# endernewton/tf-faster-rcnn

Hardware: AMD Instinct MI355X
Metric: images/sec (600×1000) ResNet-101 Faster R-CNN at 1/2/4/8 MI355X (higher is better)
Workload: dtype f32 (operands, accumulators, results; GEMMs with Cin, Cout % 128 == 0 form each f32 product from two-piece fp16 operands with an exact power-of-two scale per 128-k block on the fp16 matrix pipe -- 3 MFMAs / product, dropped terms <= 3 * 2^-22, measured error vs float64 below the f32-MFMA kernel's; o

## Files before the change

tf-faster-rcnn_amd/csrc/conv_igemm.hip:

```cpp
#include "common.h"
#include "mfma_f32.h"
#include <mutex>
#include <type_traits>

__device__ float4 g_zero_page[4];

struct ConvParams {
  const float* x; const float* w; const float* bias; const float* res; float* y;
  const float* mask;
  int N, H, W, Cin, OH, OW, Cout, KH, KW, stride, pad_top, pad_left, act;
  int RH, RW, res_stride;
  int M, Ktot, nsteps;
  int mtiles, ntiles;
  int batch;
  long long gx, gw, gy;
  int reserved;
  int splits, kchunk;
  long long gz;
  int stagger, stagger_slots;
};

__device__ __forceinline__ size_t res_offset_strided(int m, int n, int Cout, int res_stride, int ohow, int OW, int RH, int RW) {
  const int img = m / ohow, rem = m % ohow, oh = rem / OW, ow = rem % OW;
  return ((size_t)(img * RH + oh * res_stride) * RW + ow * res_stride) * Cout + n;
}

template <int TM, int TN>
__device__ __forceinline__ void frag_read(float4 (&a)[TM], const float* sb, const int& a_row0, const int& koff, float4 (&b)[TN], const int& b_row0) {
#pragma unroll
  for (int i = 0; i < TM; ++i) a[i] = *(const float4*)(sb + a_row0 + i * 1024 + koff);
#pragma unroll
  for (int j = 0; j < TN; ++j) b[j] = *(const float4*)(sb + b_row0 + j * 1024 + koff);
}
template <int TM, int TN>
__device__ __forceinline__ void frag_mfma(const float4 (&a)[TM], const float4 (&b)[TN], f32x16 (&acc2)[TM][TN], f32x16 (&acc)[TM][TN]) {
  constexpr bool KSPLIT = (TM * TN == 1);
#pragma unroll
  for (int e = 0; e < 4; ++e)
#pragma unroll
    for (int i = 0; i < TM; ++i)
#pragma unroll
      for (int j = 0; j < TN; ++j) {
        const float av = e == 0 ? a[i].x : e == 1 ? a[i].y : e == 2 ? a[i].z : a[i].w;
        const float bv = e == 0 ? b[j].x : e == 1 ? b[j].y : e == 2 ? b[j].z : b[j].w;
        if (KSPLIT && (e & 1)) acc2[i][j] = __builtin_amdgcn_mfma_f32_32x32x2f32(av, bv, acc2[i][j], 0, 0, 0);
        else acc[i][j] = __builtin_amdgcn_mfma_f32_32x32x2f32(av, bv, acc[i][j], 0, 0, 0);
      }
}

template <int BM, int BN, int WM, int WN, int NS, bool FOLDW, bool ILV = false, bool RF = false>
__global__ __launch_bounds__((BM / WM) * (BN / WN) * 64) void k_conv_igemm(const ConvParams p) {
  constexpr int NW = (BM / WM) * (BN / WN);
  constexpr int NT = NW * 64;
  constexpr int TM = WM / 32, TN = WN / 32;
  constexpr int LA = BM / 8 / NW, LB = BN / 8 / NW;
  constexpr int G = LA + LB;
  constexpr int P = NS - 1;
  constexpr int SLAB = (BM + BN) * 32;
  constexpr int EPI_LD = BN;
  static_assert((BM / 8) % NW == 0 && (BN / 8) % NW == 0, "tile/wave mismatch");
  static_assert((P - 1) * G <= 63, "vmcnt range");
  extern __shared__ __attribute__((aligned(16))) float smem[];

  const int tid = threadIdx.x, lane = tid & 63;
  const int wave = __builtin_amdgcn_readfirstlane(tid >> 6);
  if (p.stagger > 0) {
    const unsigned slot = blockIdx.x >> 8;
    if (blockIdx.y == 0 && blockIdx.z == 0 && slot > 0 && slot < (unsigned)p.stagger_slots) {
      const long long t0 = clock64(), wait = (long long)p.stagger * slot;
      while (clock64() - t0 < wait) __builtin_amdgcn_s_sleep(16);
    }
  }
  const int nwg = p.mtiles * p.ntiles;
  int bid = blockIdx.x;
  {
    const int q = nwg / 8, r = nwg % 8, xcd = bid % 8, idx = bid / 8;
    bid = (xcd < r ? xcd * (q + 1) : r * (q + 1) + (xcd - r) * q) + idx;
  }
  const int mt = bid / p.ntiles, nt = bid % p.ntiles;
  const int bm0 = mt * BM, bn0 = nt * BN;
  const int wm0 = (wave / (BN / WN)) * WM, wn0 = (wave % (BN / WN)) * WN;
  const float* const px = p.x + (size_t)blockIdx.y * p.gx;
  const float* const pw = p.w + (size_t)blockIdx.y * p.gw;
  float* const py = p.y + (size_t)blockIdx.y * p.gy + (size_t)blockIdx.z * p.gz;
  const int s_begin = (int)blockIdx.z * p.kchunk;
  const int nloc = p.splits > 1 ? min(p.nsteps - s_begin, p.kchunk) : p.nsteps;

  const int lrow = lane >> 3, lpos = lane & 7;
  int a_base[LA], a_ih0[LA], a_iw0[LA], a_q4[LA];
#pragma unroll
  for (int t = 0; t < LA; ++t) {
    const int row = (wave * LA + t) * 8 + lrow;
    a_q4[t] = (lpos ^ ((row >> 1) & 7)) * 4;
    const int m = bm0 + row;
    if (m < p.M) {
      const int img = m / (p.OH * p.OW), rem = m % (p.OH * p.OW);
      const int oh = rem / p.OW, ow = rem % p.OW;
      a_base[t] = img * p.H * p.W * p.Cin;
      a_ih0[t] = oh * p.stride - p.pad_top;
      a_iw0[t] = ow * p.stride - p.pad_left;
    } else {
      a_base[t] = 0; a_ih0[t] = -(1 << 28); a_iw0[t] = -(1 << 28);
    }
  }
  const float* zero = (const float*)g_zero_page;
  const float* a_ptr[LA]; int a_inc[LA];
  const float* b_ptr[LB]; int b_inc[LB];
#pragma unroll
  for (int t = 0; t < LB; ++t) {
    const int row = BM + (wave * LB + t) * 8 + lrow;
    const int n = bn0 + row - BM;
    const int q4 = (lpos ^ ((row >> 1) & 7)) * 4;
    const bool ok = n < p.Cout;
    b_ptr[t] = ok ? pw + (size_t)n * p.Ktot + q4 + (size_t)s_begin * 32 : zero;
    b_inc[t] = ok ? 32 : 0;
  }
  int kh = 0, kw = 0, c0 = 0;
  if (!FOLDW && s_begin) {
    const int k0 = s_begin * 32, tap = k0 / p.Cin;
    c0 = k0 - tap * p.Cin;
    kh = tap / p.KW;
    kw = tap - kh * p.KW;
  }

  auto set_tap = [&]() {
#pragma unroll
    for (int t = 0; t < LA; ++t) {
      const int ih = a_ih0[t] + kh, iw = a_iw0[t] + kw;
      bool ok = (unsigned)ih < (unsigned)p.H;
      if (FOLDW) ok = ok && ((unsigned)(iw + (a_q4[t] >> 2)) < (unsigned)p.W);
      else ok = ok && ((unsigned)iw < (unsigned)p.W);
      a_ptr[t] = ok ? px + (size_t)(a_base[t] + (ih * p.W + iw) * p.Cin + c0 + a_q4[t]) : zero;
      a_inc[t] = ok ? 32 : 0;
    }
  };
  const unsigned lds0 = (unsigned)(size_t)(LDS_AS float*)smem;
  auto issue_one = [&](int buf, int t) {
    const unsigned sb = lds0 + (unsigned)(buf * SLAB * 4);
    if (t < LA) {
      glds16(a_ptr[t], __builtin_amdgcn_readfirstlane(sb + (wave * LA + t) * 1024));
      a_ptr[t] += a_inc[t];
    } else {
      const int u = t - LA;
      glds16(b_ptr[u], __builtin_amdgcn_readfirstlane(sb + BM * 128 + (wave * LB + u) * 1024));
      b_ptr[u] += b_inc[u];
    }
  };
  auto advance_k = [&]() {
    if (FOLDW) { ++kh; }
    else {
      c0 += 32;
      if (c0 == p.Cin) { c0 = 0; if (++kw == p.KW) { kw = 0; ++kh; } }
    }
  };
  auto issue_slab = [&](int buf) {
    if (c0 == 0) set_tap();
#pragma unroll
    for (int t = 0; t < G; ++t) issue_one(buf, t);
    advance_k();
  };

  constexpr bool KSPLIT = (TM * TN == 1);
  f32x16 acc[TM][TN], acc2[TM][TN];
#pragma unroll
  for (int i = 0; i < TM; ++i)
#pragma unroll
    for (int j = 0; j < TN; ++j)
#pragma unroll
      for (int r = 0; r < 16; ++r) { acc[i][j][r] = 0.f; acc2[i][j][r] = 0.f; }

  const int frow = lane & 31, khalf = lane >> 5;
  int koff[4];
#pragma unroll
  for (int s = 0; s < 4; ++s) koff[s] = ((2 * s + khalf) ^ ((frow >> 1) & 7)) * 4;
  const int a_row0 = (wm0 + frow) * 32, b_row0 = (BM + wn0 + frow) * 32;

  if (c0 != 0) set_tap();
#pragma unroll
  for (int s = 0; s < P; ++s)
    if (s < nloc) issue_slab(s);

  auto slab = [&](auto more_c, int step) {
    constexpr bool MORE = decltype(more_c)::value;
    if (MORE || step + P <= nloc) wait_vmcnt<(P - 1) * G>();
    else wait_vmcnt<0>();
    __builtin_amdgcn_s_barrier();
    const int nbuf = (step + P) % NS;
    const float* sb = smem + (step % NS) * SLAB;
    float4 a[4][TM], b[4][TN];
    auto read_frag = [&](int q) { frag_read(a[q], sb, a_row0, koff[q], b[q], b_row0); };
    auto mfma_group = [&](int q) { frag_mfma(a[q], b[q], acc2, acc); };
    if (ILV) {
      if (MORE && c0 == 0) set_tap();
      read_frag(0);
#pragma unroll
      for (int q = 0; q < 4; ++q) {
        if (q < 3) read_frag(q + 1);
        if (MORE) {
#pragma unroll
          for (int t = (q * G) / 4; t < ((q + 1) * G) / 4; ++t) issue_one(nbuf, t);
        }
        mfma_group(q);
      }
      if (MORE) advance_k();
    } else {
      constexpr int RF_FIRST = !RF ? 0 : (TM * TN == 1 ? 4 : 1);
#pragma unroll
      for (int q = 0; q < RF_FIRST; ++q) read_frag(q);
      if (MORE) issue_slab(nbuf);
#pragma unroll
      for (int q = RF_FIRST; q < 4; ++q) read_frag(q);
      if (TM * TN == 1) __builtin_amdgcn_sched_barrier(0);
#pragma unroll
      for (int q = 0; q < 4; ++q) mfma_group(q);
    }
  };
  {
    int step = 0;
    for (; step + P < nloc; ++step) slab(std::true_type{}, step);
    for (; step < nloc; ++step) slab(std::false_type{}, step);
  }
  if (KSPLIT) {
#pragma unroll
    for (int i = 0; i < TM; ++i)
#pragma unroll
      for (int j = 0; j < TN; ++j)
#pragma unroll
        for (int r = 0; r < 16; ++r) acc[i][j][r] += acc2[i][j][r];
  }

  __syncthreads();
#pragma unroll
  for (int i = 0; i < TM; ++i)
#pragma unroll
    for (int j = 0; j < TN; ++j)
#pragma unroll
      for (int r = 0; r < 16; ++r) {
        const int ml = wm0 + i * 32 + (r & 3) + 8 * (r >> 2) + 4 * khalf;
        smem[ml * EPI_LD + wn0 + j * 32 + frow] = acc[i][j][r];
      }
  __syncthreads();
  const int ohow = p.OH * p.OW;
  if ((p.Cout & 3) == 0) {
    constexpr int C4 = BN / 4;
    for (int t = tid; t < BM * C4; t += NT) {
      const int ml = t / C4, nl = (t % C4) * 4;
      const int m = bm0 + ml, n = bn0 + nl;
      if (m >= p.M || n >= p.Cout) continue;
      float4 v = *(const float4*)(smem + ml * EPI_LD + nl);
      if (p.bias) {
        const float4 bv = *(const float4*)(p.bias + n);
        v.x += bv.x; v.y += bv.y; v.z += bv.z; v.w += bv.w;
      }
      if (p.res) {
        size_t ro;
        if (p.res_stride == 1) ro = (size_t)m * p.Cout + n;
        else ro = res_offset_strided(m, n, p.Cout, p.res_stride, ohow, p.OW, p.RH, p.RW);
        const float4 rv = *(const float4*)(p.res + ro);
        v.x += rv.x; v.y += rv.y; v.z += rv.z; v.w += rv.w;
      }
      if (p.act == FRCNN_ACT_RELU) v = act_relu(v);
      else if (p.act == FRCNN_ACT_RELU6)
        v = act_relu6(v);
      if (p.mask) {
        const float4 k = *(const float4*)(p.mask + (size_t)m * p.Cout + n);
        v.x = k.x > 0.f ? v.x : 0.f; v.y = k.y > 0.f ? v.y : 0.f; v.z = k.z > 0.f ? v.z : 0.f; v.w = k.w > 0.f ? v.w : 0.f;
      }
      *(float4*)(py + (size_t)m * p.Cout + n) = v;
    }
  } else {
    for (int t = tid; t < BM * BN; t += NT) {
      const int ml = t / BN, nl = t % BN;
      const int m = bm0 + ml, n = bn0 + nl;
      if (m >= p.M || n >= p.Cout) continue;
      float v = smem[ml * EPI_LD + nl] + (p.bias ? p.bias[n] : 0.f);
      if (p.res) {
        size_t ro;
        if (p.res_stride == 1) ro = (size_t)m * p.Cout + n;
        else ro = res_offset_strided(m, n, p.Cout, p.res_stride, ohow, p.OW, p.RH, p.RW);
        v += p.res[ro];
      }
      if (p.act == FRCNN_ACT_RELU) v = act_relu(v);
      else if (p.act == FRCNN_ACT_RELU6) v = act_relu6(v);
      if (p.mask) v = p.mask[(size_t)m * p.Cout + n] > 0.f ? v : 0.f;
      py[(size_t)m * p.Cout + n] = v;
    }
  }
}

template <int BM, int BN, int WM, int WN, int NS, bool FOLDW, bool ILV = false, bool RF = false>
static int launch_conv(ConvParams p, hipStream_t st) {
  constexpr int NT = (BM / WM) * (BN / WN) * 64;
  constexpr size_t ring = sizeof(float) * NS * (BM + BN) * 32, epi = sizeof(float) * BM * BN;
  constexpr size_t lds = ring > epi ? ring : epi;
  auto kern = k_conv_igemm<BM, BN, WM, WN, NS, FOLDW, ILV, RF>;
  static KernelOnce once;
  HIP_TRY(kernel_once(once, (const void*)kern, NT, lds));
  p.mtiles = cdiv(p.M, BM);
  p.ntiles = cdiv(p.Cout, BN);
  hipLaunchKernelGGL(kern, dim3(p.mtiles * p.ntiles, p.batch, p.splits), dim3(NT), lds, st, p);
  LAUNCH_CHECK();
  return FRCNN_OK;
}

struct GemmParams {
  const float* x; const float* w; const float* bias; const float* res; float* y;
  int M, N, K, nsteps, mtiles, ntiles, batch, act;
  long long gx, gw, gy;
};

template <int BM, int BN, int WM, int WN, bool ILV, bool RF, bool RESPF>
__global__ __launch_bounds__((BM / WM) * (BN / WN) * 64) void k_gemm_stream(const GemmParams p) {
  constexpr int NW = (BM / WM) * (BN / WN);
  constexpr int TM = WM / 32, TN = WN / 32;
  constexpr int LA = BM / 8 / NW, LB = BN / 8 / NW;
  constexpr int G = LA + LB;
  constexpr int SLAB = (BM + BN) * 32;
  static_assert((BM / 8) % NW == 0 && (BN / 8) % NW == 0, "tile/wave mismatch");
  extern __shared__ __attribute__((aligned(16))) float smem[];

  const int tid = threadIdx.x, lane = tid & 63;
  const int wave = __builtin_amdgcn_readfirstlane(tid >> 6);
  const int per = p.mtiles * p.ntiles, T = per * p.batch;
  const int xcd = blockIdx.x & 7, wx = blockIdx.x >> 3, W8 = gridDim.x >> 3;
  const int tq = T / 8, tr = T % 8, tn = tq + (xcd < tr ? 1 : 0);
  const int t_end = (xcd < tr ? xcd * (tq + 1) : tr * (tq + 1) + (xcd - tr) * tq) + tn;
  int tile = __builtin_amdgcn_readfirstlane(t_end - tn + wx);
  if (tile >= t_end) return;

  const int wm0 = (wave / (BN / WN)) * WM, wn0 = (wave % (BN / WN)) * WN;
  const int lrow = lane >> 3, lpos = lane & 7;
  int a_lane[LA], b_lane[LB];
#pragma unroll
  for (int t = 0; t < LB; ++t) {
    const int row = (wave * LB + t) * 8 + lrow;
    b_lane[t] = row * p.K + (lpos ^ (((BM + row) >> 1) & 7)) * 4;
  }
  const float* ia = p.x; const float* ib = p.w;
  int i_bm0 = 0, i_bn0 = 0, i_g = 0;
  auto set_tile = [&](int tl) {
    const int g = tl / per, rem = tl - g * per;
    const int mt = rem / p.ntiles, nt = rem - mt * p.ntiles;
    i_bm0 = mt * BM; i_bn0 = nt * BN; i_g = g;
    ia = p.x + (size_t)g * p.gx + (size_t)i_bm0 * p.K;
    ib = p.w + (size_t)g * p.gw + (size_t)i_bn0 * p.K;
#pragma unroll
    for (int t = 0; t < LA; ++t) {
      const int row = (wave * LA + t) * 8 + lrow;
      a_lane[t] = (min(row, p.M - 1 - i_bm0)) * p.K + (lpos ^ ((row >> 1) & 7)) * 4;
    }
  };
  const unsigned lds0 = (unsigned)(size_t)(LDS_AS float*)smem;
  auto issue_one = [&](int buf, int t) {
    const unsigned sb = lds0 + (unsigned)(buf * SLAB * 4);
    if (t < LA) glds16(ia + a_lane[t], __builtin_amdgcn_readfirstlane(sb + (wave * LA + t) * 1024));
    else glds16(ib + b_lane[t - LA], __builtin_amdgcn_readfirstlane(sb + BM * 128 + (wave * LB + (t - LA)) * 1024));
  };
  auto advance_k = [&]() { ia += 32; ib += 32; };
  auto issue_slab = [&](int buf) {
#pragma unroll
    for (int t = 0; t < G; ++t) issue_one(buf, t);
    advance_k();
  };

  constexpr bool KSPLIT = (TM * TN == 1);
  f32x16 acc[TM][TN], acc2[TM][TN];
  auto zero_acc = [&]() {
#pragma unroll
    for (int i = 0; i < TM; ++i)
#pragma unroll
      for (int j = 0; j < TN; ++j)
#pragma unroll
        for (int r = 0; r < 16; ++r) { acc[i][j][r] = 0.f; acc2[i][j][r] = 0.f; }
  };
  zero_acc();
  const int frow = lane & 31, khalf = lane >> 5;
  int koff[4];
#pragma unroll
  for (int s = 0; s < 4; ++s) koff[s] = ((2 * s + khalf) ^ ((frow >> 1) & 7)) * 4;
  const int a_row0 = (wm0 + frow) * 32, b_row0 = (BM + wn0 + frow) * 32;

  int c_bm0, c_bn0, c_g;
  float rv[RESPF ? TM : 1][RESPF ? TN : 1][16];
  const int lane_off = (4 * khalf * p.N + frow) * 4;
  auto sub_base = [&](int i, int j) { return (long long)(c_bm0 + wm0 + i * 32) * p.N + (long long)(c_bn0 + wn0 + j * 32); };
  auto row_soff = [&](int r) { return ((r & 3) + 8 * (r >> 2)) * p.N * 4; };
  auto rsrc_of = [&](const float* tensor, long long sbase) {
    const long long left = ((long long)p.M * p.N - sbase) * 4;
    return __builtin_amdgcn_make_buffer_rsrc((void*)(tensor + sbase), 0, (int)max(0ll, min(left, 0x7fffffffll)), 0x00020000);
  };
  auto prefetch_res = [&]() {
    if (!RESPF || !p.res) return;
    int lo = lane_off;
    asm volatile("" : "+v"(lo));
#pragma unroll
    for (int i = 0; i < TM; ++i)
#pragma unroll
      for (int j = 0; j < TN; ++j) {
        const auto rr = rsrc_of(p.res + (size_t)c_g * p.gy, sub_base(i, j));
#pragma unroll
        for (int r = 0; r < 16; ++r) rv[RESPF ? i : 0][RESPF ? j : 0][r] = __builtin_bit_cast(float, __builtin_amdgcn_raw_buffer_load_b32(rr, lo + row_soff(r), 0, 0));
      }
  };

  auto slab_body = [&](int cur) {
    const int nbuf = cur ^ 1;
    const float* sb = smem + cur * SLAB;
    float4 a[4][TM], b[4][TN];
    auto read_frag = [&](int q) { frag_read(a[q], sb, a_row0, koff[q], b[q], b_row0); };
    auto mfma_group = [&](int q) { frag_mfma(a[q], b[q], acc2, acc); };
    if (ILV) {
      read_frag(0);
#pragma unroll
      for (int q = 0; q < 4; ++q) {
        if (q < 3) read_frag(q + 1);
#pragma unroll
        for (int t = (q * G) / 4; t < ((q + 1) * G) / 4; ++t) issue_one(nbuf, t);
        mfma_group(q);
      }
      advance_k();
    } else {
      constexpr int RF_FIRST = !RF ? 0 : (TM * TN == 1 ? 4 : 1);
#pragma unroll
      for (int q = 0; q < RF_FIRST; ++q) read_frag(q);
      issue_slab(nbuf);
#pragma unroll
      for (int q = RF_FIRST; q < 4; ++q) read_frag(q);
      if (TM * TN == 1) __builtin_amdgcn_sched_barrier(0);
#pragma unroll
      for (int q = 0; q < 4; ++q) mfma_group(q);
    }
  };

  const float act_lo = p.act == FRCNN_ACT_NONE ? -__builtin_inff() : 0.f;
  const float act_hi = p.act == FRCNN_ACT_RELU6 ? 6.f : __builtin_inff();
  auto finish = [&](auto res_c) {
    constexpr bool RES = decltype(res_c)::value;
    float* const py = p.y + (size_t)c_g * p.gy;
    int lo = lane_off;
    asm volatile("" : "+v"(lo));
#pragma unroll
    for (int i = 0; i < TM; ++i)
#pragma unroll
      for (int j = 0; j < TN; ++j) {
        const float bv = p.bias ? p.bias[c_bn0 + wn0 + j * 32 + frow] : 0.f;
        const long long sbase = sub_base(i, j);
        float v[16];
        if (RES && !RESPF) {
          const auto rr = rsrc_of(p.res + (size_t)c_g * p.gy, sbase);
#pragma unroll
          for (int r = 0; r < 16; ++r) v[r] = __builtin_bit_cast(float, __builtin_amdgcn_raw_buffer_load_b32(rr, lo + row_soff(r), 0, 0));
        }
#pragma unroll
        for (int r = 0; r < 16; ++r) {
          float t = (KSPLIT ? acc[i][j][r] + acc2[i][j][r] : acc[i][j][r]) + bv;
          if (RES) t += RESPF ? rv[RESPF ? i : 0][RESPF ? j : 0][r] : v[r];
          v[r] = act_clamp(t, act_lo, act_hi);
        }
        const auto ry = rsrc_of(py, sbase);
#pragma unroll
        for (int r = 0; r < 16; ++r) __builtin_amdgcn_raw_buffer_store_b32(__builtin_bit_cast(unsigned, v[r]), ry, lo + row_soff(r), 0, 0);
      }
  };

  set_tile(tile);
  c_bm0 = i_bm0; c_bn0 = i_bn0; c_g = i_g;
  issue_slab(0);
  int cur = 0, step = 0;
  for (;;) {
    wait_vmcnt<0>();
    __builtin_amdgcn_s_barrier();
    const bool last = step + 1 == p.nsteps;
    int next = tile;
    if (last) {
      next = __builtin_amdgcn_readfirstlane(tile + W8);
      set_tile(next < t_end ? next : tile);
      prefetch_res();
    }
    slab_body(cur);
    cur ^= 1;
    if (!last) { ++step; continue; }
    if (p.res) finish(std::true_type{}); else finish(std::false_type{});
    if (next >= t_end) break;
    zero_acc();
    step = 0; tile = next; c_bm0 = i_bm0; c_bn0 = i_bn0; c_g = i_g;
  }
  wait_vmcnt<0>();
}

template <int BM, int BN, int WM, int WN, bool ILV, bool RF, bool RESPF>
static int launch_stream(const ConvParams& c, hipStream_t st) {
  constexpr int NT = (BM / WM) * (BN / WN) * 64;
  constexpr size_t lds = sizeof(float) * 2 * (BM + BN) * 32;
  auto kern = k_gemm_stream<BM, BN, WM, WN, ILV, RF, RESPF>;
  static KernelOnce once;
  int slots = 0;
  HIP_TRY(kernel_once(once, (const void*)kern, NT, lds, &slots));
  const bool plain = c.KH == 1 && c.KW == 1 && c.stride == 1 && c.pad_top == 0 && c.pad_left == 0 && c.OH == c.H && c.OW == c.W;
  if (slots < 8 || !plain || c.mask || c.Cout % BN || c.splits != 1 || (c.res && c.res_stride != 1) || (long long)c.M * c.Cout >= (1ll << 31) ||
      (long long)c.M * c.Cin >= (1ll << 31) || (long long)c.Cout * c.Cin >= (1ll << 31))
    return FRCNN_E_UNSUPPORTED;
  GemmParams p;
  p.x = c.x; p.w = c.w; p.bias = c.bias; p.res = c.res; p.y = c.y;
  p.mtiles = cdiv(c.M, BM); p.M = c.M; p.N = c.Cout; p.K = c.Cin; p.nsteps = c.Cin / 32;
  p.ntiles = c.Cout / BN; p.batch = c.batch; p.act = c.act;
  p.gx = c.gx; p.gw = c.gw; p.gy = c.gy;
  const long long T = (long long)p.mtiles * p.ntiles * p.batch;
  if (T >= (1ll << 30)) return FRCNN_E_UNSUPPORTED;
  const int grid = (int)min((long long)(slots / 8) * 8, ((T + 7) / 8) * 8);
  hipLaunchKernelGGL(kern, dim3(grid), dim3(NT), lds, st, p);
  LAUNCH_CHECK();
  return FRCNN_OK;
}

enum : int {
  IGEMM_64x32_NS4 = 4,
  IGEMM_64x64_ILV = 15,
  IGEMM_128_RF = 20,
  IGEMM_128_8W_RF = 21,
  STREAM_64x64 = 100, STREAM_64x64_RESPF = 101,
  STREAM_128_RF = 102,
  STREAM_128_8W_RF = 104, STREAM_128_8W_RF_RESPF = 105,
  STREAM_128x64 = 106, STREAM_128x64_RESPF = 107,
  STREAM_64x128 = 108, STREAM_64x128_RESPF = 109,
  STREAM_128x64_4W_RESPF = 110, STREAM_64x128_4W_RESPF = 111,
  STREAM_32x64 = 112,
  STREAM_32x128 = 114,
};

static int launch_cfg(int id, const ConvParams& p, hipStream_t st) {
  switch (id) {
    case IGEMM_64x32_NS4: return launch_conv<64, 32, 32, 32, 4, false>(p, st);
    case IGEMM_64x64_ILV: return launch_conv<64, 64, 32, 32, 2, false, true>(p, st);
    case IGEMM_128_RF: return launch_conv<128, 128, 64, 64, 2, false, false, true>(p, st);
    case IGEMM_128_8W_RF: return launch_conv<128, 128, 32, 64, 2, false, false, true>(p, st);
    case STREAM_64x64: return launch_stream<64, 64, 32, 32, true, false, false>(p, st);
    case STREAM_64x64_RESPF: return launch_stream<64, 64, 32, 32, true, false, true>(p, st);
    case STREAM_128_RF: return launch_stream<128, 128, 64, 64, false, true, false>(p, st);
    case STREAM_128_8W_RF: return launch_stream<128, 128, 32, 64, false, true, false>(p, st);
    case STREAM_128_8W_RF_RESPF: return launch_stream<128, 128, 32, 64, false, true, true>(p, st);
    case STREAM_128x64: return launch_stream<128, 64, 32, 32, true, false, false>(p, st);
    case STREAM_128x64_RESPF: return launch_stream<128, 64, 32, 32, true, false, true>(p, st);
    case STREAM_64x128: return launch_stream<64, 128, 32, 32, true, false, false>(p, st);
    case STREAM_64x128_RESPF: return launch_stream<64, 128, 32, 32, true, false, true>(p, st);
    case STREAM_128x64_4W_RESPF: return launch_stream<128, 64, 64, 32, false, true, true>(p, st);
    case STREAM_64x128_4W_RESPF: return launch_stream<64, 128, 32, 64, false, true, true>(p, st);
    case STREAM_32x64: return launch_stream<32, 64, 32, 32, true, false, false>(p, st);
    case STREAM_32x128: return launch_stream<32, 128, 32, 32, true, false, false>(p, st);
    default: return FRCNN_E_ARG;
  }
}

static thread_local int g_force_cfg = -1, g_stagger = 0, g_stream = 1, g_split_target = 640;
static thread_local int g_plan_images = 0;
static constexpr int PLAN_IMAGES = 4;
extern thread_local int g_wino_rows_below;
extern "C" int frcnn_set_tuning(int key, int value) {
  if (key == 9) { g_wino_rows_below = value > 0 ? value : 256; return FRCNN_OK; }
  if (key == 0) { g_force_cfg = value; return FRCNN_OK; }
  if (key == 5) { g_stagger = value; return FRCNN_OK; }
  if (key == 6) { g_stream = value; return FRCNN_OK; }
  if (key == 7) { g_split_target = value > 0 ? value : 640; return FRCNN_OK; }
  if (key == 8) { g_plan_images = value > 0 ? value : 0; return FRCNN_OK; }
  return FRCNN_E_ARG;
}

static long long plan_rows(long long M) {
  return (g_plan_images > 0 && M % g_plan_images == 0) ? M / g_plan_images * PLAN_IMAGES : M;
}

static long long tiles_128(long long rows, int Cout, int groups) { return (rows + 127) / 128 * cdiv(Cout, 128) * groups; }

static int tile_cfg_64(int Cout) { return Cout > 32 ? IGEMM_64x64_ILV : IGEMM_64x32_NS4; }
static int tile_cfg(long long rows, int Cout, int nsteps, int groups) {
  if (Cout >= 96 && tiles_128(rows, Cout, groups) >= 384 && nsteps >= 8) return Cout >= 1024 ? IGEMM_128_8W_RF : IGEMM_128_RF;
  return tile_cfg_64(Cout);
}

static bool short_k_stream(long long rows, int Cout, int nsteps, int groups) {
  return g_stream && nsteps <= 8 && Cout % 128 == 0 && (rows + 63) / 64 * (Cout / 128) * groups >= 512;
}

static int plan_splits(int M, int Cout, int nsteps) {
  if (g_force_cfg >= 0) return 1;
  M = (int)min(plan_rows(M), (long long)0x7fffffff);
  if (tile_cfg(M, Cout, nsteps, 1) != tile_cfg_64(Cout)) return 1;
  const long long tiles = (long long)cdiv(M, 64) * cdiv(Cout, Cout > 32 ? 64 : 32);
  if (tiles >= 384 || nsteps < 16) return 1;
  int S = (int)min((long long)8, (g_split_target + tiles - 1) / tiles);
  S = min(S, nsteps / 8);
  if (S < 2) return 1;
  const int kchunk = cdiv(nsteps, S);
  return cdiv(nsteps, kchunk);
}

extern "C" size_t frcnn_conv2d_workspace_bytes(int N, int OH, int OW, int Cout, int KH, int KW, int Cin, int fold_w) {
  if (fold_w || N <= 0 || OH <= 0 || OW <= 0 || Cout <= 0 || KH <= 0 || KW <= 0 || Cin <= 0 || Cin % 32) return 0;
  const long long M = (long long)N * OH * OW;
  if (M >= (1ll << 29)) return 0;
  const int S = plan_splits((int)M, Cout, KH * KW * (Cin / 32));
  return S > 1 ? (size_t)S * (size_t)M * (size_t)Cout * sizeof(float) : 0;
}

__global__ void k_splitk_finish(const float* __restrict__ part, int S, int M, int Cout, const float* __restrict__ bias,
                                const float* res, int res_stride, int OH, int OW, int RH, int RW, int act, const float* __restrict__ mask,
                                float* y) {
  const long long total = (long long)M * Cout;
  const int ohow = OH * OW;
  for (long long i = (long long)blockIdx.x * blockDim.x + threadIdx.x; i < total; i += (long long)gridDim.x * blockDim.x) {
    float v = part[i];
    for (int s = 1; s < S; ++s) v += part[(size_t)s * total + i];
    const int m = (int)(i / Cout), n = (int)(i - (long long)m * Cout);
    if (bias) v += bias[n];
    if (res) {
      size_t ro;
      if (res_stride == 1) ro = (size_t)i;
      else ro = res_offset_strided(m, n, Cout, res_stride, ohow, OW, RH, RW);
      v += res[ro];
    }
    if (act == FRCNN_ACT_RELU) v = act_relu(v);
    else if (act == FRCNN_ACT_RELU6) v = act_relu6(v);
    if (mask) v = mask[i] > 0.f ? v : 0.f;
    y[i] = v;
  }
}

static ConvParams conv_params() {
  ConvParams p = {};
  p.KH = p.KW = p.stride = p.res_stride = p.batch = p.splits = 1;
  p.act = FRCNN_ACT_NONE;
  return p;
}

static int conv2d_impl(const float* x_d, int N, int H, int W, int Cin, const float* w_d, const float* bias_d,
                       const float* residual_d, int RH, int RW, int res_stride, float* y_d, int OH, int OW, int Cout, int KH, int KW,
                       int stride, int pad_top, int pad_left, int act, int fold_w, void* ws, size_t ws_bytes, const float* mask_d,
                       void* stream) {
  if (!x_d || !w_d || !y_d) return FRCNN_E_ARG;
  if (N <= 0 || H <= 0 || W <= 0 || Cin <= 0 || OH <= 0 || OW <= 0 || Cout <= 0 || KH <= 0 || KW <= 0 || stride <= 0)
    return FRCNN_E_ARG;
  if (act < 0 || act > 2) return FRCNN_E_ARG;
  if (residual_d && (res_stride < 1 || RH < (OH - 1) * res_stride + 1 || RW < (OW - 1) * res_stride + 1)) return FRCNN_E_ARG;
  if (fold_w) {
    if (Cin != 4 || KW > 8) return FRCNN_E_UNSUPPORTED;
  } else if (Cin % 32) {
    return FRCNN_E_UNSUPPORTED;
  }
  if ((long long)N * H * W * Cin >= (1ll << 31) || (long long)N * OH * OW >= (1ll << 31) / 4) return FRCNN_E_UNSUPPORTED;
  ConvParams p = conv_params();
  p.x = x_d; p.w = w_d; p.bias = bias_d; p.res = residual_d; p.y = y_d; p.mask = mask_d;
  p.N = N; p.H = H; p.W = W; p.Cin = Cin; p.OH = OH; p.OW = OW; p.Cout = Cout; p.KH = KH; p.KW = fold_w ? 1 : KW;
  p.stride = stride; p.pad_top = pad_top; p.pad_left = pad_left; p.act = act;
  p.RH = RH; p.RW = RW; p.res_stride = residual_d ? res_stride : 1;
  p.M = N * OH * OW;
  p.Ktot = fold_w ? KH * 32 : KH * KW * Cin;
  p.nsteps = p.kchunk = fold_w ? KH : KH * KW * (Cin / 32);
  hipStream_t st = (hipStream_t)stream;
  if (fold_w) return launch_conv<128, 64, 32, 64, 3, true>(p, st);
  if (g_force_cfg >= 0) return launch_cfg(g_force_cfg, p, st);
  const long long Mp = plan_rows(p.M);
  if (ws) {
    const int S = plan_splits(p.M, Cout, p.nsteps);
    if (S > 1 && (size_t)S * p.M * Cout * sizeof(float) <= ws_bytes) {
      ConvParams q = p;
      q.bias = nullptr; q.res = nullptr; q.act = FRCNN_ACT_NONE; q.y = (float*)ws; q.mask = nullptr;
      q.kchunk = cdiv(p.nsteps, S); q.splits = S; q.gz = (long long)p.M * Cout;
      const int rc = launch_cfg(tile_cfg_64(Cout), q, st);
      if (rc) return rc;
      const long long total = (long long)p.M * Cout;
      hipLaunchKernelGGL(k_splitk_finish, dim3((unsigned)min((long long)2048, (total + 255) / 256)), dim3(256), 0, st, (const float*)ws, S,
                         p.M, Cout, bias_d, residual_d, p.res_stride, OH, OW, RH, RW, act, mask_d, y_d);
      LAUNCH_CHECK();
      return FRCNN_OK;
    }
  }
  if (stride == 1 && KH == 1 && KW == 1 && (!residual_d || p.res_stride == 1)) {
    int rc = FRCNN_E_UNSUPPORTED;
    if (short_k_stream(Mp, Cout, p.nsteps, 1)) rc = launch_cfg(STREAM_64x128, p, st);
    else if (g_stream && p.nsteps <= 8 && Cout == 64 && (Mp + 127) / 128 >= 512) rc = launch_cfg(STREAM_128x64, p, st);
    if (rc != FRCNN_E_UNSUPPORTED) return rc;
  }
  const int cfg = tile_cfg(Mp, Cout, p.nsteps, 1);
  if (cfg != tile_cfg_64(Cout)) {
    if (g_stagger > 0 && tiles_128(Mp, Cout, 1) >= 1024) {
      p.stagger = (int)min((long long)p.nsteps * 8192 * g_stagger / 8, (long long)1 << 30);
      p.stagger_slots = 2;
    }
  } else if (g_stagger > 0 && (g_stagger & 16) && Cout > 32 && (long long)cdiv(p.M, 64) * cdiv(Cout, 64) >= 1280) {
    p.stagger = p.nsteps * 1024;
    p.stagger_slots = 5;
  }
  return launch_cfg(cfg, p, st);
}

extern "C" int frcnn_conv2d_nhwc(const float* x_d, int N, int H, int W, int Cin, const float* w_d, const float* bias_d,
                                 const float* residual_d, int RH, int RW, int res_stride, float* y_d, int OH, int OW,
                                 int Cout, int KH, int KW, int stride, int pad_top, int pad_left, int act, int fold_w,
                                 void* stream) {
  return conv2d_impl(x_d, N, H, W, Cin, w_d, bias_d, residual_d, RH, RW, res_stride, y_d, OH, OW, Cout, KH, KW, stride, pad_top,
                     pad_left, act, fold_w, nullptr, 0, nullptr, stream);
}

extern "C" int frcnn_conv2d_nhwc_ws(const float* x_d, int N, int H, int W, int Cin, const float* w_d, const float* bias_d,
                                    const float* residual_d, int RH, int RW, int res_stride, float* y_d, int OH, int OW,
                                    int Cout, int KH, int KW, int stride, int pad_top, int pad_left, int act, int fold_w,
                                    void* ws, size_t ws_bytes, void* stream) {
  return conv2d_impl(x_d, N, H, W, Cin, w_d, bias_d, residual_d, RH, RW, res_stride, y_d, OH, OW, Cout, KH, KW, stride, pad_top,
                     pad_left, act, fold_w, ws, ws_bytes, nullptr, stream);
}

extern "C" int frcnn_conv2d_nhwc_masked_ws(const float* x_d, int N, int H, int W, int Cin, const float* w_d, const float* bias_d,
                                           const float* residual_d, int RH, int RW, int res_stride, float* y_d, int OH, int OW,
                                           int Cout, int KH, int KW, int stride, int pad_top, int pad_left, int act, const float* mask_d,
                                           void* ws, size_t ws_bytes, void* stream) {
  if (!mask_d) return FRCNN_E_ARG;
  return conv2d_impl(x_d, N, H, W, Cin, w_d, bias_d, residual_d, RH, RW, res_stride, y_d, OH, OW, Cout, KH, KW, stride, pad_top,
                     pad_left, act, 0, ws, ws_bytes, mask_d, stream);
}

extern "C" int frcnn_gemm_batched_nt(const float* x_d, const float* w_d, float* y_d, int G, int M, int N, int K, void* stream) {
  if (!x_d || !w_d || !y_d || G <= 0 || M <= 0 || N <= 0 || K <= 0) return FRCNN_E_ARG;
  if (K % 32 || G > 65535) return FRCNN_E_UNSUPPORTED;
  ConvParams p = conv_params();
  p.x = x_d; p.w = w_d; p.y = y_d;
  p.N = 1; p.H = 1; p.W = M; p.Cin = K; p.OH = 1; p.OW = M; p.Cout = N;
  p.M = M; p.Ktot = K; p.nsteps = p.kchunk = K / 32;
  p.gx = (long long)M * K; p.gw = (long long)N * K; p.gy = (long long)M * N;
  p.batch = G;
  hipStream_t st = (hipStream_t)stream;
  if (g_force_cfg >= 0) return launch_cfg(g_force_cfg, p, st);
  const long long Mp = plan_rows(M);
  if (short_k_stream(Mp, N, p.nsteps, G)) {
    const int rc = launch_cfg(STREAM_64x128, p, st);
    if (rc != FRCNN_E_UNSUPPORTED) return rc;
  }
  const bool waste = (Mp + 127) / 128 * 128 * 4 > Mp * 5;
  return launch_cfg(waste ? tile_cfg_64(N) : tile_cfg(Mp, N, p.nsteps, G), p, st);
}

extern "C" int frcnn_pack_filter_hwio(const float* w_hwio, int KH, int KW, int Cin, int Cout, const float* scale, float* out) {
  if (!w_hwio || !out || KH <= 0 || KW <= 0 || Cin <= 0 || Cout <= 0) return FRCNN_E_ARG;
  for (int kh = 0; kh < KH; ++kh)
    for (int kw = 0; kw < KW; ++kw)
      for (int c = 0; c < Cin; ++c) {
        const float* src = w_hwio + (((size_t)kh * KW + kw) * Cin + c) * Cout;
        for (int o = 0; o < Cout; ++o)
          out[(((size_t)o * KH + kh) * KW + kw) * Cin + c] = scale ? src[o] * scale[o] : src[o];
      }
  return FRCNN_OK;
}
```

Baseline: 555.4.

## Add dedicated stem convolution kernel with LDS-resident weights and per-wave pipelined tiles

Adds a specialised kernel for the folded-width stem convolution (Cin=4 packed, small Cout). The whole filter stays resident in LDS, and each wave streams 32-row activation tiles through a 3-slot async-load ring spread across XCD-partitioned tiles, running f32 MFMAs with a fused bias and activation epilogue. It is meant to replace the generic 128x64 implicit-GEMM path, which wastes tile width and pipeline depth on this tiny-Cout layer. The old path stays available through a tuning key and as a fallback when the new kernel rejects the shape.

Result: no change. 554.4 (-0.2%).

```diff
diff --git a/tf-faster-rcnn_amd/csrc/conv_igemm.hip b/tf-faster-rcnn_amd/csrc/conv_igemm.hip
--- a/tf-faster-rcnn_amd/csrc/conv_igemm.hip
+++ b/tf-faster-rcnn_amd/csrc/conv_igemm.hip
@@ -513,6 +513,197 @@
   return FRCNN_OK;
 }
 
+constexpr int STEM_NW = 8, STEM_NS = 3;
+
+template <int NCH, int TN>
+__global__ __launch_bounds__(STEM_NW * 64) void k_stem_fold(const ConvParams p) {
+  constexpr int P = STEM_NS - 1, LA = 4;
+  constexpr int NFULL = NCH / 2, NG = (NCH + 1) / 2;
+  extern __shared__ __attribute__((aligned(16))) float smem[];
+  const int tid = threadIdx.x, lane = tid & 63;
+  const int wave = __builtin_amdgcn_readfirstlane(tid >> 6);
+  const int KH = p.KH, FROWS = TN * 32;
+  const int lrow = lane >> 3, lpos = lane & 7;
+  const float* zero = (const float*)g_zero_page;
+  const unsigned lds0 = (unsigned)(size_t)(LDS_AS float*)smem;
+
+  for (int blk = wave; blk < KH * FROWS / 8; blk += STEM_NW) {
+    const int row = blk * 8 + lrow, kh = row / FROWS, n = row % FROWS;
+    const float* src = n < p.Cout ? p.w + (size_t)n * p.Ktot + kh * 32 + (lpos ^ ((n >> 1) & 7)) * 4 : zero;
+    glds16(src, __builtin_amdgcn_readfirstlane(lds0 + blk * 1024));
+  }
+
+  const int T = (p.M + 31) / 32;
+  const int xcd = blockIdx.x & 7, wx = blockIdx.x >> 3, W8 = gridDim.x >> 3;
+  const int tq = T / 8, tr = T % 8, tn = tq + (xcd < tr ? 1 : 0);
+  const int t_end = (xcd < tr ? xcd * (tq + 1) : tr * (tq + 1) + (xcd - tr) * tq) + tn;
+  const int stride = W8 * STEM_NW;
+  int tile = __builtin_amdgcn_readfirstlane(t_end - tn + wave * W8 + wx);
+
+  const unsigned ohow = (unsigned)(p.OH * p.OW), uOH = (unsigned)p.OH, uOW = (unsigned)p.OW;
+  const unsigned dm = (unsigned)stride * 32u, d_img = dm / ohow, d_oh = dm % ohow / uOW, d_ow = dm % ohow % uOW;
+  unsigned r_img[LA], r_oh[LA], r_ow[LA];
+  int a_off[LA], a_ih0[LA]; bool a_ok[LA];
+  int i_tile = tile, i_kh = 0, i_slot = 0;
+  auto set_rows = [&]() {
+#pragma unroll
+    for (int t = 0; t < LA; ++t) {
+      const int pix = lpos ^ (((t * 8 + lrow) >> 1) & 7);
+      const int iw = (int)r_ow[t] * p.stride - p.pad_left + pix;
+      a_ih0[t] = (int)r_oh[t] * p.stride - p.pad_top;
+      a_ok[t] = i_tile < t_end && r_img[t] < (unsigned)p.N && (unsigned)iw < (unsigned)p.W;
+      a_off[t] = (int)(((r_img[t] * (unsigned)p.H + (unsigned)a_ih0[t]) * (unsigned)p.W + (unsigned)iw) * 4u);
+    }
+  };
+  auto next_tile = [&]() {
+    i_tile += stride;
+#pragma unroll
+    for (int t = 0; t < LA; ++t) {
+      unsigned ow = r_ow[t] + d_ow, oh = r_oh[t] + d_oh;
+      if (ow >= uOW) { ow -= uOW; ++oh; }
+      r_ow[t] = ow;
+      r_img[t] += d_img;
+      if (oh >= uOH) { oh -= uOH; ++r_img[t]; }
+      r_oh[t] = oh;
+    }
+    set_rows();
+  };
+#pragma unroll
+  for (int t = 0; t < LA; ++t) {
+    const unsigned m = (unsigned)tile * 32u + t * 8 + lrow, rem = m % ohow;
+    r_img[t] = m / ohow; r_oh[t] = rem / uOW; r_ow[t] = rem % uOW;
+  }
+  const unsigned ring0 = lds0 + (unsigned)(KH * FROWS * 128 + wave * STEM_NS * 4096);
+  auto issue_next = [&]() {
+    const unsigned sb = ring0 + (unsigned)(i_slot * 4096);
+    const int koffs = i_kh * p.W * 4;
+#pragma unroll
+    for (int t = 0; t < LA; ++t) {
+      const bool ok = a_ok[t] && (unsigned)(a_ih0[t] + i_kh) < (unsigned)p.H;
+      glds16(ok ? p.x + (a_off[t] + koffs) : zero, __builtin_amdgcn_readfirstlane(sb + t * 1024));
+    }
+    i_slot = i_slot == STEM_NS - 1 ? 0 : i_slot + 1;
+    if (++i_kh == KH) { i_kh = 0; next_tile(); }
+  };
+  set_rows();
+#pragma unroll
+  for (int s = 0; s < P; ++s) issue_next();
+  wait_vmcnt<0>();
+  __syncthreads();
+  if (tile >= t_end) return;
+
+  const int frow = lane & 31, khalf = lane >> 5, sw = (frow >> 1) & 7;
+  int koff[NG];
+#pragma unroll
+  for (int s = 0; s < NG; ++s) koff[s] = ((s < NFULL ? 2 * s + khalf : 2 * s) ^ sw) * 4;
+  float* const ring = smem + KH * FROWS * 32 + wave * STEM_NS * 1024;
+
+  constexpr int LD = TN * 32, RP = 32 / TN, C4 = LD / 4, RR = 16 / TN;
+  const int e_nl = (lane % C4) * 4, e_ml = lane / C4;
+  float4 bv = make_float4(-0.f, -0.f, -0.f, -0.f);
+  if (p.bias && e_nl < p.Cout) bv = *(const float4*)(p.bias + e_nl);
+  const float act_lo = p.act == FRCNN_ACT_NONE ? -__builtin_inff() : 0.f;
+  const float act_hi = p.act == FRCNN_ACT_RELU6 ? 6.f : __builtin_inff();
+
+  int c_slot = 0;
+  for (;;) {
+    f32x16 acc[TN];
+#pragma unroll
+    for (int j = 0; j < TN; ++j)
+#pragma unroll
+      for (int r = 0; r < 16; ++r) acc[j][r] = 0.f;
+    float* slot = ring;
+    for (int kh = 0; kh < KH; ++kh) {
+      wait_vmcnt<(P - 1) * LA>();
+      slot = ring + c_slot * 1024;
+      const float* fa = slot + frow * 32;
+      const float* fb = smem + kh * (FROWS * 32) + frow * 32;
+      float4 a[NG], b[NG][TN];
+#pragma unroll
+      for (int s = 0; s < NG; ++s) {
+        a[s] = *(const float4*)(fa + koff[s]);
+#pragma unroll
+        for (int j = 0; j < TN; ++j) b[s][j] = *(const float4*)(fb + j * 1024 + koff[s]);
+      }
+      issue_next();
+#pragma unroll
+      for (int s = 0; s < NFULL; ++s)
+#pragma unroll
+        for (int e = 0; e < 4; ++e)
+#pragma unroll
+          for (int j = 0; j < TN; ++j) {
+            const float av = e == 0 ? a[s].x : e == 1 ? a[s].y : e == 2 ? a[s].z : a[s].w;
+            const float bw = e == 0 ? b[s][j].x : e == 1 ? b[s][j].y : e == 2 ? b[s][j].z : b[s][j].w;
+            acc[j] = __builtin_amdgcn_mfma_f32_32x32x2f32(av, bw, acc[j], 0, 0, 0);
+          }
+      if constexpr (NCH & 1) {
+#pragma unroll
+        for (int e = 0; e < 2; ++e)
+#pragma unroll
+          for (int j = 0; j < TN; ++j) {
+            const float4 av = a[NFULL], bw = b[NFULL][j];
+            acc[j] = __builtin_amdgcn_mfma_f32_32x32x2f32(e == 0 ? (khalf ? av.y : av.x) : (khalf ? av.w : av.z),
+                                                          e == 0 ? (khalf ? bw.y : bw.x) : (khalf ? bw.w : bw.z), acc[j], 0, 0, 0);
+          }
+      }
+      c_slot = c_slot == STEM_NS - 1 ? 0 : c_slot + 1;
+    }
+#pragma unroll
+    for (int h = 0; h < TN; ++h) {
+#pragma unroll
+      for (int j = 0; j < TN; ++j)
+#pragma unroll
+        for (int rr = 0; rr < RR; ++rr) {
+          const int r = h * RR + rr;
+          slot[((r & 3) + 8 * (r >> 2) - h * RP + 4 * khalf) * LD + j * 32 + frow] = acc[j][r];
+        }
+      __builtin_amdgcn_fence(__ATOMIC_RELEASE, "wavefront");
+      __builtin_amdgcn_wave_barrier();
+      __builtin_amdgcn_fence(__ATOMIC_ACQUIRE, "wavefront");
+      float4 v[4];
+#pragma unroll
+      for (int i = 0; i < 4; ++i) v[i] = *(const float4*)(slot + (e_ml + i * (64 / C4)) * LD + e_nl);
+#pragma unroll
+      for (int i = 0; i < 4; ++i) {
+        const int m = tile * 32 + h * RP + e_ml + i * (64 / C4);
+        v[i].x = act_clamp(v[i].x + bv.x, act_lo, act_hi); v[i].y = act_clamp(v[i].y + bv.y, act_lo, act_hi);
+        v[i].z = act_clamp(v[i].z + bv.z, act_lo, act_hi); v[i].w = act_clamp(v[i].w + bv.w, act_lo, act_hi);
+        if (m < p.M && e_nl < p.Cout) *(float4*)(p.y + (size_t)m * p.Cout + e_nl) = v[i];
+      }
+      __builtin_amdgcn_fence(__ATOMIC_RELEASE, "wavefront");
+      __builtin_amdgcn_wave_barrier();
+      __builtin_amdgcn_fence(__ATOMIC_ACQUIRE, "wavefront");
+    }
+    tile += stride;
+    if (tile >= t_end) break;
+  }
+  wait_vmcnt<0>();
+}
+
+template <int NCH, int TN>
+static int launch_stem_fold(const ConvParams& p, hipStream_t st) {
+  constexpr size_t lds_max = 160 * 1024;
+  const size_t lds = sizeof(float) * ((size_t)p.KH * TN * 1024 + STEM_NW * STEM_NS * 1024);
+  if (lds > lds_max) return FRCNN_E_UNSUPPORTED;
+  auto kern = k_stem_fold<NCH, TN>;
+  static KernelOnce once;
+  int slots = 0;
+  HIP_TRY(kernel_once(once, (const void*)kern, STEM_NW * 64, lds_max, &slots));
+  if (slots < 8) return FRCNN_E_UNSUPPORTED;
+  const int T = cdiv(p.M, 32);
+  const int grid = min(slots / 8 * 8, 8 * cdiv(T, 8));
+  hipLaunchKernelGGL(kern, dim3(grid), dim3(STEM_NW * 64), lds, st, p);
+  LAUNCH_CHECK();
+  return FRCNN_OK;
+}
+
+static int launch_stem(const ConvParams& p, int KW, hipStream_t st) {
+  if (p.Cout > 64 || (p.Cout & 3) || p.res || p.mask) return FRCNN_E_UNSUPPORTED;
+  if (KW == 7 && p.Cout > 32) return launch_stem_fold<7, 2>(p, st);
+  if (KW == 3 && p.Cout <= 32) return launch_stem_fold<3, 1>(p, st);
+  return launch_stem_fold<8, 2>(p, st);
+}
+
 enum : int {
   IGEMM_64x32_NS4 = 4,
   IGEMM_64x64_ILV = 15,
@@ -554,6 +745,7 @@
 static thread_local int g_force_cfg = -1, g_stagger = 0, g_stream = 1, g_split_target = 640;
 static thread_local int g_plan_images = 0;
 static constexpr int PLAN_IMAGES = 4;
+static thread_local int g_stem_igemm = 0;
 extern thread_local int g_wino_rows_below;
 extern "C" int frcnn_set_tuning(int key, int value) {
   if (key == 9) { g_wino_rows_below = value > 0 ? value : 256; return FRCNN_OK; }
@@ -562,6 +754,7 @@
   if (key == 6) { g_stream = value; return FRCNN_OK; }
   if (key == 7) { g_split_target = value > 0 ? value : 640; return FRCNN_OK; }
   if (key == 8) { g_plan_images = value > 0 ? value : 0; return FRCNN_OK; }
+  if (key == 10) { g_stem_igemm = value == 1; return FRCNN_OK; }
   return FRCNN_E_ARG;
 }
 
@@ -656,7 +849,10 @@
   p.Ktot = fold_w ? KH * 32 : KH * KW * Cin;
   p.nsteps = p.kchunk = fold_w ? KH : KH * KW * (Cin / 32);
   hipStream_t st = (hipStream_t)stream;
-  if (fold_w) return launch_conv<128, 64, 32, 64, 3, true>(p, st);
+  if (fold_w) {
+    const int rc = g_stem_igemm ? FRCNN_E_UNSUPPORTED : launch_stem(p, KW, st);
+    return rc != FRCNN_E_UNSUPPORTED ? rc : launch_conv<128, 64, 32, 64, 3, true>(p, st);
+  }
   if (g_force_cfg >= 0) return launch_cfg(g_force_cfg, p, st);
   const long long Mp = plan_rows(p.M);
   if (ws) {
```
